# songrise/HyperNeRF-torch

Hardware: NVIDIA B200
Metric: train rays/s (fwd+bwd, 64+64 samples/ray, HyperNeRF warp+bendy-sheet) (higher is better)
Workload: dtype bf16

## Files before the change

hypernerf_torch_b200/csrc/hn_mlp.cu:

```cuda
#include <math.h>
#include <algorithm>
#include <string.h>
#include <type_traits>
#include <unordered_map>
#include "hn_api_internal.h"
#include "hn_mlp_program.h"
#include "hn_ptx.cuh"

#ifdef HN_MLP_FWD_VARIANT
namespace hn_fv { using namespace hn; }
#define hn hn_fv
#define hn_mlp_fwd hn_mlp_fwd_fv
#define hn_mlp_fwd_trunk hn_mlp_fwd_trunk_fv
#define HN_FV_HIDDEN __attribute__((visibility("hidden")))
#else
#define HN_FV_HIDDEN
#endif

namespace hn {

#ifndef HN_TRAP_IDS
#define HN_TRAP_IDS 1
#endif
#if HN_TRAP_IDS
// ... 806 lines not shown
          tc_fence_before();
          warp_arrive(my_ready);
        }
#if HN_ROLE_TIMING
        if (p.dbg && blockIdx.x == 0 && threadIdx.x == 0) {
          p.dbg[gridDim.x * 8 + li * 2] += t_drain - t_layer;
          p.dbg[gridDim.x * 8 + li * 2 + 1] += HN_T0() - t_drain;
        }
#endif
        (void)t_layer; (void)t_drain;
      }
    }
    if (p.dbg && threadIdx.x == 0) {
      const long long tt = HN_T0() - t_begin;
      p.dbg[blockIdx.x * 8 + 4] = t_acc; p.dbg[blockIdx.x * 8 + 5] = tt - t_acc - t_pro;
      p.dbg[blockIdx.x * 8 + 6] = t_pro; p.dbg[blockIdx.x * 8 + 7] = tt;
    }
    };
    if (kEpiSplit == 1 || share == 0) { setmaxnreg_inc<kRegsPrimary>(); epilogue(std::true_type{}); }
    else { setmaxnreg_dec<kRegsSecondary>(); epilogue(std::false_type{}); }
  }
  tc_fence_before();
  __syncthreads();
  if (warp == kIssuerWarp) tmem_dealloc(tmem_base, 256 * kSubTiles);
}

template <class C>
__device__ __forceinline__ void trunk_in_bwd(uint32_t tlane, const float* wp, float* gx) {
  if constexpr (C::KT <= 96) {
    float gf[C::KT];
#pragma unroll
    for (int c0 = 0; c0 < C::KT; c0 += 32) {
      uint32_t r[32];
      tmem_ld32(tlane + c0, r);
      tmem_ld_wait();
#pragma unroll
      for (int j = 0; j < 32; ++j) gf[c0 + j] = __uint_as_float(r[j]);
    }
    posenc_bwd<3, C::XF>(wp, gf, gx);
    if constexpr (C::H > 0) posenc_bwd<C::H, C::HF>(wp + 3, gf + C::PE_X, gx + 3);
  } else {
    static_assert(C::PE_X == 63, "the two-phase pull-back assumes the hyper block starts at column 63");
    float gh[C::PE_H + 8];
    {
      float ga[64];
#pragma unroll
      for (int c0 = 0; c0 < 64; c0 += 32) {
        uint32_t r[32];
        tmem_ld32(tlane + c0, r);
        tmem_ld_wait();
#pragma unroll
        for (int j = 0; j < 32; ++j) ga[c0 + j] = __uint_as_float(r[j]);
      }
      posenc_bwd<3, C::XF>(wp, ga, gx);
      gh[0] = ga[63];
    }
#pragma unroll
    for (int c0 = 64; c0 < C::KT; c0 += 16) {
      uint32_t r[16];
      tmem_ld16(tlane + c0, r);
      tmem_ld_wait();
#pragma unroll
      for (int j = 0; j < 16; ++j)
        if (c0 - 63 + j < C::PE_H) gh[c0 - 63 + j] = __uint_as_float(r[j]);
    }
    posenc_bwd<C::H, C::HF>(wp + 3, gh, gx + 3);
  }
}

template <class C>
__global__ void __launch_bounds__(kMlpThreads, 1) mlp_dgrad_kernel(const __grid_constant__ BwdParams p) {
  extern __shared__ __align__(1024) uint8_t smem[];
  using SM = SmemBwd<C>;
  using Ring = RingStateT<SM::STAGES>;
  constexpr bool PP = true;
  uint8_t* act = smem + SM::ACT;
  uint8_t* inb = smem + SM::INB;
  uint8_t* ring = smem + SM::RING;
  uint64_t* full = reinterpret_cast<uint64_t*>(smem + SM::BARS);
  uint64_t* empty = full + SM::STAGES;
  uint64_t* acc_full = empty + SM::STAGES;
  uint64_t* act_ready = acc_full + 2;
  uint32_t* tmem_ptr = reinterpret_cast<uint32_t*>(smem + SM::TMEMP);
  const int warp = threadIdx.x >> 5, lane = threadIdx.x & 31;

  if (threadIdx.x == 0) {
    for (int i = 0; i < SM::STAGES; ++i) { mbar_init(&full[i], 1); mbar_init(&empty[i], 1); }
    for (int i = 0; i < 2; ++i) { mbar_init(&acc_full[i], 1); mbar_init(&act_ready[i], 4 * Sched<PP>::SUBS * kEpiSplit); }
    fence_barrier_init();
  }
  if (warp == kIssuerWarp) { tmem_alloc(tmem_ptr, 256 * kSubTiles); tmem_relinquish(); }
  tc_fence_before();
  __syncthreads();
  tc_fence_after();
  const uint32_t tmem_base = *tmem_ptr;
  const Program& prog = p.prog;

  if (warp >= kEpiWarps) {
    setmaxnreg_dec<kRegsFeeder>();
    if (warp == kProducerWarp && lane == 0) {
      Ring rs;
      long long tw = 0;
      for (int tile = blockIdx.x; tile < p.n_tiles; tile += gridDim.x) produce_tile<PP>(prog, p.weights, ring, full, empty, rs, tw);
      if (p.dbg) p.dbg[blockIdx.x * 8 + 0] = tw;
    } else if (warp == kIssuerWarp) {
      Ring rs;
      uint32_t ph_ready = 0;
      long long t_ready = 0, t_full = 0;
      const long long t_begin = HN_T0();
      const uint32_t act_s = smem_u32(act), inb_s = smem_u32(inb), ring_s = smem_u32(ring);
      for (int tile = blockIdx.x; tile < p.n_tiles; tile += gridDim.x) {
        for (int li = 0; li < prog.nlayers; ++li) {
          for (int chain = 0; chain < Sched<PP>::CHAINS; ++chain) {
            long long t0 = HN_T0();
            mbar_wait(&act_ready[chain], ph_ready);
            t_ready += HN_T0() - t0;
            tc_fence_after();
            issue_layer<PP>(prog, prog.layers[li], chain * Sched<PP>::SUBS, act_s, inb_s, SM::ACT_BYTES, SM::INB_BYTES, ring_s, tmem_base,
                        full, empty, rs, t_full);
            if (elect_one_sync()) umma_commit(&acc_full[chain]);
            __syncwarp();
          }
          ph_ready ^= 1;
        }
      }
      if (p.dbg && lane == 0) {
        p.dbg[blockIdx.x * 8 + 1] = t_ready; p.dbg[blockIdx.x * 8 + 2] = t_full; p.dbg[blockIdx.x * 8 + 3] = HN_T0() - t_begin;
      }
    }
  } else {
    const int sub = warp / (4 * kEpiSplit);
    const int share = (warp >> 2) % kEpiSplit;
    const int quarter = warp & 3;
    auto epilogue = [&](auto primary_tag) {
    constexpr bool PRIMARY = decltype(primary_tag)::value;
    const int row = quarter * 32 + lane;
    const uint32_t tlane = tmem_base + ((uint32_t)(quarter * 32) << 16) + sub * 256;
    uint8_t* act_row = act + sub * SM::ACT_BYTES + row * 16;
    uint8_t* inb_row = inb + sub * SM::INB_BYTES + row * 16;
    const int chain = PP ? sub : 0;
    uint64_t* my_acc = &acc_full[chain];
    uint64_t* my_ready = &act_ready[chain];
    uint32_t ph_acc = 0;
    long long t_acc = 0, t_pro = 0;
    const long long t_begin = HN_T0();
    for (int tile = blockIdx.x; tile < p.n_tiles; tile += gridDim.x) {
      const long long t_tile = HN_T0();
      const int64_t g = (int64_t)tile * kCtaRows + sub * kTileRows + row;
      const bool valid = g < p.n;
      const int64_t gc = valid ? g : p.n - 1;
      const int64_t ray = gc / p.S;
      const int64_t gq = p.pos != nullptr ? ray * p.S_full + __ldg(p.pos + gc) : gc;
      const size_t half = (size_t)tile * (2 * kSubTiles) + sub * 2 + (row >> 6);
      const uint32_t* gate_row = p.gates + half * (size_t)p.g_total * kHalfRows + (row & 63);
      uint4* save_row = reinterpret_cast<uint4*>(p.dsaved + half * (size_t)p.d_total * kHalfChunkBytes) + (row & 63);

      if constexpr (PRIMARY) {
        float f[16];
#pragma unroll
        for (int i = 0; i < 16; ++i) f[i] = 0.f;
        if (valid) {
#pragma unroll
          for (int i = 0; i < 3; ++i) {
            float y = __ldg(p.rgb + gq * 3 + i);
            f[i] = __ldg(p.g_rgb + gq * 3 + i) * y * (1.f - y);
          }
        }
        store_features<16>(f, act_row, save_row, p.d_rgbhead);
        if constexpr (C::STATIC) {
#pragma unroll
          for (int i = 0; i < 16; ++i) f[i] = 0.f;
          if (valid && __ldg(p.sigma + gq) > 0.f) f[0] = __ldg(p.g_sigma + gq);
          store_features<16>(f, inb_row, save_row, p.d_sigma);
        }
      }
      fence_proxy_async_smem();
      tc_fence_before();
      warp_arrive(my_ready);
      t_pro += HN_T0() - t_tile;

      float gx_skip[C::STATIC ? 1 : C::NWARPED] = {};
      for (int li = 0; li < prog.nlayers; ++li) {
        const Layer& L = prog.layers[li];
        if (L.epi == BE_MASK) {
          if (L.n_out == kTrunkW) bwd_masked_share<kTrunkW>(share, tlane, gate_row, L.gate_word, act_row, save_row, L.save_chunk, my_acc, ph_acc, t_acc);
          else if (L.n_out == kWsW) bwd_masked_share<kWsW>(share, tlane, gate_row, L.gate_word, act_row, save_row, L.save_chunk, my_acc, ph_acc, t_acc);
          else bwd_masked_share<kRgbW>(share, tlane, gate_row, L.gate_word, act_row, save_row, L.save_chunk, my_acc, ph_acc, t_acc);
          fence_proxy_async_smem();
          if (li + 1 < prog.nlayers) { tc_fence_before(); warp_arrive(my_ready); }
          continue;
        }
        if (!C::STATIC && L.epi == BE_RGB1) {
          bwd_masked_share<kRgbW>(share, tlane, gate_row, L.gate_word, act_row, save_row, L.save_chunk, my_acc, ph_acc, t_acc);
          if constexpr (PRIMARY) {
          float f[16];
#pragma unroll
          for (int i = 0; i < 16; ++i) f[i] = 0.f;
          if (valid) f[0] = __ldg(p.g_sigma + gq) * (-expm1f(-__ldg(p.sigma + gq)));
          store_features<16>(f, act_row + (kRgbW / 8) * kChunkBytes, save_row, L.save_chunk + kRgbW / 8);
          }
          fence_proxy_async_smem(); tc_fence_before(); warp_arrive(my_ready);
          continue;
        }
        { long long t0 = HN_T0(); mbar_wait(my_acc, ph_acc); ph_acc ^= 1; t_acc += HN_T0() - t0; }
        tc_fence_after();
        if (L.epi == BE_LINEAR || L.epi == BE_LINCOND) {
          if (L.n_out == kTrunkW) bwd_linear_share<kTrunkW>(share, tlane, act_row, save_row, L.save_chunk);
          else bwd_linear_share<kRgbW>(share, tlane, act_row, save_row, L.save_chunk);
          if constexpr (PRIMARY && !C::STATIC) {
            if (L.epi == BE_LINCOND) {
              uint32_t r[16];
              tmem_ld16(tlane + kRgbW, r);
              tmem_ld_wait();
              float v[C::G];
#pragma unroll
              for (int i = 0; i < C::G; ++i) v[i] = __uint_as_float(r[i]);
              const int64_t id = __ldg(p.ids + ray);
              HN_CHECK_ID(id, p.n_embed);
              glo_grad_add<C::G>(v, valid, id, p.glo_grad, lane);
            }
          }
        } else if constexpr (PRIMARY && !C::STATIC) {
        if (L.epi == BE_SKIPSTORE || L.epi == BE_TRUNKIN) {
          float wp[C::NWARPED], gx[C::NWARPED];
          const int64_t gw = p.g_warped_out != nullptr ? gc : gq;
#pragma unroll
          for (int i = 0; i < C::NWARPED; ++i) wp[i] = __ldg(p.warped + gw * C::NWARPED + i);
          trunk_in_bwd<C>(tlane, wp, gx);
          if (L.epi == BE_SKIPSTORE) {
#pragma unroll
            for (int i = 0; i < C::NWARPED; ++i) gx_skip[i] = gx[i];
          } else if (p.g_warped_out != nullptr) {
            if (valid) {
#pragma unroll
              for (int i = 0; i < C::NWARPED; ++i) {
                float v = gx[i] + gx_skip[i];
                if (p.g_warped != nullptr) v += __ldg(p.g_warped + gq * C::NWARPED + i);
                p.g_warped_out[g * C::NWARPED + i] = v;
              }
            }
          } else if constexpr (!C::NOWARP) {
          float f[16];
#pragma unroll
          for (int i = 0; i < 16; ++i) f[i] = 0.f;
          if (valid) {
#pragma unroll
            for (int i = 0; i < C::NWARPED; ++i) {
              f[i] = gx[i] + gx_skip[i];
              if (p.g_warped != nullptr) f[i] += __ldg(p.g_warped + gq * C::NWARPED + i);
            }
          }
          if constexpr (C::H == C::G) {
            if (p.mflags & MF_AXIS) {
              const int64_t id = __ldg(p.ids + ray);
              glo_grad_add<C::G>(f + 3, valid, id, p.glo_grad, lane);
#pragma unroll
              for (int i = 0; i < C::G; ++i) f[3 + i] = 0.f;
            }
          }
          if constexpr (C::SE3) {
            float x[3], wv[6], gy[3];
#pragma unroll
            for (int i = 0; i < 3; ++i) { x[i] = __ldg(p.points + gq * 3 + i); gy[i] = f[i]; }
#pragma unroll
            for (int i = 0; i < 6; ++i) wv[i] = __ldg(p.aux + gc * 6 + i);
            se3_apply_bwd(x, wv, wv + 3, gy, f, f + 3);
          }
          store_features<16>(f, act_row, save_row, L.save_chunk);
          }
        } else if constexpr (!C::NOWARP) {
          uint32_t r[16];
          tmem_ld16(tlane + kWsW, r);
          tmem_ld_wait();
          float v[C::G];
#pragma unroll
          for (int i = 0; i < C::G; ++i) v[i] = __uint_as_float(r[i]);
          const int64_t id = __ldg(p.ids + ray);
          HN_CHECK_ID(id, p.n_embed);
          glo_grad_add<C::G>(v, valid, id, p.glo_grad, lane);
        }
        }
        if (li + 1 < prog.nlayers) {
          fence_proxy_async_smem();
          tc_fence_before();
          warp_arrive(my_ready);
        }
      }
    }
    if (p.dbg && threadIdx.x == 0) {
      const long long tt = HN_T0() - t_begin;
      p.dbg[blockIdx.x * 8 + 4] = t_acc; p.dbg[blockIdx.x * 8 + 5] = tt - t_acc - t_pro;
      p.dbg[blockIdx.x * 8 + 6] = t_pro; p.dbg[blockIdx.x * 8 + 7] = tt;
    }
    };
    if (kEpiSplit == 1 || share == 0) { setmaxnreg_inc<kRegsPrimary>(); epilogue(std::true_type{}); }
    else { setmaxnreg_dec<kRegsSecondary>(); epilogue(std::false_type{}); }
  }
  tc_fence_before();
  __syncthreads();
  if (warp == kIssuerWarp) tmem_dealloc(tmem_base, 256 * kSubTiles);
}

#ifndef HN_MLP_FWD_VARIANT
constexpr int kWgStages = 3;
constexpr int kWgStageA = 256 * kHalfChunkBytes / 8;
constexpr int kWgStageBytes = 2 * kWgStageA;
struct WgSmem {
  static constexpr int STAGES = 0;
  static constexpr int BARS = kWgStages * kWgStageBytes;
  static constexpr int TMEMP = BARS + (2 * kWgStages + 2) * 8;
  static constexpr int TOTAL = TMEMP + 16;
};
static int wgrad_groups(int njobs) { return njobs >= 24 ? 8 : 4; }
static void assign_wgrad_groups(WgradTable& t, int groups, int grid, int16_t* group_start) {
  int order[kMaxJobs];
  int64_t load[16] = {};
  auto cost = [&](int i) { return (int)t.jobs[i].dy_nchunks + t.jobs[i].x0_nchunks + t.jobs[i].x1_nchunks; };
  for (int i = 0; i < t.njobs; ++i) order[i] = i;
  std::stable_sort(order, order + t.njobs, [&](int a, int b) { return cost(a) > cost(b); });
  for (int k = 0; k < t.njobs; ++k) {
    int best = 0;
    for (int g = 1; g < groups; ++g) if (load[g] < load[best]) best = g;
    t.jobs[order[k]].group = (uint8_t)best;
    load[best] += cost(order[k]);
  }
  int ctas[16];
  for (int g = 0; g < groups; ++g) ctas[g] = 1;
  for (int c = groups; c < grid; ++c) {
    int best = 0;
    for (int g = 1; g < groups; ++g)
      if (load[g] * ctas[best] > load[best] * ctas[g]) best = g;
    ++ctas[best];
  }
  group_start[0] = 0;
  for (int g = 0; g < groups; ++g) group_start[g + 1] = (int16_t)(group_start[g] + ctas[g]);
}

__device__ __forceinline__ float pe_window(float alpha, uint8_t win_c, int e) {
  const int C = win_c & ~kWinIdentity;
  if (win_c & kWinIdentity) {
    if (e < C) return 1.f;
    e -= C;
  }
  const float x = fminf(fmaxf(alpha - (float)(e / (2 * C)), 0.f), 1.f);
  return 0.5f * (1.f - cospif(x));
}

struct WgradParams {
  WgradTable tab;
  const uint8_t* saved; const uint8_t* dsaved;
  const float* pe_alpha;
  float* flat_grad;
  int64_t n_half;
  int x_total, d_total;
  int groups;
  int16_t group_start[17];
};

template <bool WIN>
__global__ void __launch_bounds__(192, 1) mlp_wgrad_kernel(const __grid_constant__ WgradParams p) {
  extern __shared__ __align__(1024) uint8_t smem[];
  uint64_t* full = reinterpret_cast<uint64_t*>(smem + WgSmem::BARS);
  uint64_t* empty = full + kWgStages;
  uint64_t* acc_full = empty + kWgStages;
  uint64_t* acc_empty = acc_full + 1;
  uint32_t* tmem_ptr = reinterpret_cast<uint32_t*>(smem + WgSmem::TMEMP);
  const int warp = threadIdx.x >> 5, lane = threadIdx.x & 31;
  if (threadIdx.x == 0) {
    for (int i = 0; i < kWgStages; ++i) { mbar_init(&full[i], 1); mbar_init(&empty[i], 1 + 4); }
    mbar_init(acc_full, 1);
    mbar_init(acc_empty, 128);
    fence_barrier_init();
  }
  if (warp == 1) { tmem_alloc(tmem_ptr, 512); tmem_relinquish(); }
  tc_fence_before();
  __syncthreads();
  tc_fence_after();
  const uint32_t tmem_base = *tmem_ptr;

  int my_group = 0;
  while (my_group + 1 < p.groups && (int)blockIdx.x >= p.group_start[my_group + 1]) ++my_group;
  const int ctas_in_group = p.group_start[my_group + 1] - p.group_start[my_group];
  const int64_t per = (p.n_half + ctas_in_group - 1) / ctas_in_group;
  const int64_t h0 = (int64_t)((int)blockIdx.x - p.group_start[my_group]) * per;
  const int64_t h1 = min(h0 + per, p.n_half);
  const int njobs = p.tab.njobs;

  if (warp == 0) {
    if (lane == 0 && h0 < h1) {
      int slot = 0; uint32_t phase = 0;
      for (int ji = 0; ji < njobs; ++ji) {
        const WgradJob& J = p.tab.jobs[ji];
        if (J.group != my_group) continue;
        const uint32_t a_bytes = J.dy_nchunks * kHalfChunkBytes;
        const uint32_t b0_bytes = J.x0_nchunks * kHalfChunkBytes, b1_bytes = J.x1_nchunks * kHalfChunkBytes;
        for (int64_t h = h0; h < h1; ++h) {
          uint8_t* st = smem + slot * kWgStageBytes;
          mbar_wait(&empty[slot], phase ^ 1);
          mbar_arrive_expect_tx(&full[slot], a_bytes + b0_bytes + b1_bytes);
          bulk_g2s(st, p.dsaved + ((size_t)h * p.d_total + J.dy_chunk) * kHalfChunkBytes, a_bytes, &full[slot]);
          bulk_g2s(st + kWgStageA, p.saved + ((size_t)h * p.x_total + J.x0_chunk) * kHalfChunkBytes, b0_bytes, &full[slot]);
          if (b1_bytes)
            bulk_g2s(st + kWgStageA + b0_bytes, p.saved + ((size_t)h * p.x_total + J.x1_chunk) * kHalfChunkBytes, b1_bytes,
                       &full[slot]);
          if (++slot == kWgStages) { slot = 0; phase ^= 1; }
        }
      }
    }
  } else if (warp == 1) {
    if (h0 < h1) {
      int slot = 0; uint32_t phase = 0, ph_empty = 0;
      constexpr uint32_t kHi = (1u << 14) | (kHalfChunkBytes >> 4);
      const uint32_t st0 = smem_u32(smem);
      bool first = true;
      for (int ji = 0; ji < njobs; ++ji) {
        const WgradJob& J = p.tab.jobs[ji];
        if (J.group != my_group) continue;
        const uint32_t ncols = (J.x0_nchunks + J.x1_nchunks) * 8;
        const uint32_t idesc = make_idesc_bf16(128, ncols, 1, 1);
        const bool two = J.mblocks == 2;
        const uint32_t d1 = tmem_base + ncols;
        if (!first) { mbar_wait(acc_empty, ph_empty); ph_empty ^= 1; tc_fence_after(); }
        first = false;
        for (int64_t h = h0; h < h1; ++h) {
          mbar_wait(&full[slot], phase);
          tc_fence_after();
          if (elect_one_sync()) {
            const uint32_t a_lo = ((st0 + slot * kWgStageBytes) >> 4) | ((128u >> 4) << 16);
            const uint32_t b_lo = a_lo + (kWgStageA >> 4);
            uint32_t acc = h > h0;
#pragma unroll
            for (int ks = 0; ks < kHalfRows / 16; ++ks) {
              const uint64_t bd = ((uint64_t)kHi << 32) | (b_lo + ks * 16);
              umma_bf16(tmem_base, ((uint64_t)kHi << 32) | (a_lo + ks * 16), bd, idesc, acc);
              if (two) umma_bf16(d1, ((uint64_t)kHi << 32) | (a_lo + ks * 16 + ((16 * kHalfChunkBytes) >> 4)), bd, idesc, acc);
              acc = 1;
            }
            umma_commit(&empty[slot]);
          }
          __syncwarp();
          if (++slot == kWgStages) { slot = 0; phase ^= 1; }
        }
        if (elect_one_sync()) umma_commit(acc_full);
        __syncwarp();
      }
    }
  } else if (h0 < h1) {
    const int quarter = warp & 3;
    const int wr = warp - 2;
    const uint32_t tlane = tmem_base + ((uint32_t)(quarter * 32) << 16);
    int slot = 0; uint32_t phase = 0, ph_acc = 0;
    for (int ji = 0; ji < njobs; ++ji) {
      const WgradJob& J = p.tab.jobs[ji];
      if (J.group != my_group) continue;
      const int ncols = (J.x0_nchunks + J.x1_nchunks) * 8;
      const int cpw = (J.dy_nchunks + 3) / 4;
      const int c_lo = min(wr * cpw, (int)J.dy_nchunks), c_hi = min(c_lo + cpw, (int)J.dy_nchunks);
      float bs[8][8];
#pragma unroll
      for (int a = 0; a < 8; ++a)
#pragma unroll
        for (int b = 0; b < 8; ++b) bs[a][b] = 0.f;
      for (int64_t h = h0; h < h1; ++h) {
        mbar_wait(&full[slot], phase);
        if (J.nbias) {
          const uint8_t* st = smem + slot * kWgStageBytes;
#pragma unroll
          for (int a = 0; a < 8; ++a) {
            if (c_lo + a < c_hi) {
#pragma unroll
              for (int rr = 0; rr < kHalfRows; rr += 32) {
                uint4 v = *reinterpret_cast<const uint4*>(st + (c_lo + a) * kHalfChunkBytes + (rr + lane) * 16);
                bs[a][0] += bf16_lo(v.x); bs[a][1] += bf16_hi(v.x); bs[a][2] += bf16_lo(v.y); bs[a][3] += bf16_hi(v.y);
                bs[a][4] += bf16_lo(v.z); bs[a][5] += bf16_hi(v.z); bs[a][6] += bf16_lo(v.w); bs[a][7] += bf16_hi(v.w);
              }
            }
          }
        }
        __syncwarp();
        if (lane == 0) mbar_arrive(&empty[slot]);
        if (++slot == kWgStages) { slot = 0; phase ^= 1; }
      }
      if (J.nbias) {
#pragma unroll
        for (int a = 0; a < 8; ++a) {
          if (c_lo + a < c_hi) {
#pragma unroll
            for (int b = 0; b < 8; ++b) {
              float v = bs[a][b];
#pragma unroll
              for (int o = 16; o > 0; o >>= 1) v += __shfl_xor_sync(0xffffffffu, v, o);
              const int col = (c_lo + a) * 8 + b;
              if (lane == 0) {
                for (int s = 0; s < J.nbias; ++s) {
                  const BiasSeg& B = J.bias[s];
                  if (col >= B.col0 && col < B.col0 + B.ncols) atomicAdd(p.flat_grad + B.dst + (col - B.col0), v);
                }
              }
            }
          }
        }
      }
      mbar_wait(acc_full, ph_acc); ph_acc ^= 1;
      tc_fence_after();
      for (int mb = 0; mb < J.mblocks; ++mb) {
        const int drow = mb * 128 + quarter * 32 + lane;
        for (int c0 = 0; c0 < ncols; c0 += 16) {
          uint32_t r[16];
          tmem_ld16(tlane + mb * ncols + c0, r);
          tmem_ld_wait();
          for (int s = 0; s < J.nflush; ++s) {
            const FlushSeg& F = J.flush[s];
            if (drow >= F.row0 && drow < F.row0 + F.nrows) {
              float* dst = p.flat_grad + F.dst + (int64_t)(drow - F.row0) * F.ld + (c0 - (int)F.col0);
              const bool vec = (reinterpret_cast<uintptr_t>(dst) & 15) == 0;
              uint32_t v[16];
#pragma unroll
              for (int j = 0; j < 16; ++j) v[j] = r[j];
              if (WIN && F.win != kNoWin) {
                const float a = p.pe_alpha[F.win - 1];
#pragma unroll
                for (int j = 0; j < 16; ++j)
                  v[j] = __float_as_uint(__uint_as_float(r[j]) * pe_window(a, F.win_c, (int)F.win_e0 + c0 + j - (int)F.col0));
              }
#pragma unroll
              for (int j = 0; j < 16; j += 4) {
                const int col = c0 + j;
                if (vec && col >= F.col0 && col + 4 <= F.col0 + F.ncols) {
                  red_add_v4(dst + j, v[j], v[j + 1], v[j + 2], v[j + 3]);
                } else {
#pragma unroll
                  for (int jj = j; jj < j + 4; ++jj)
                    if (c0 + jj >= F.col0 && c0 + jj < F.col0 + F.ncols) atomicAdd(dst + jj, __uint_as_float(v[jj]));
                }
              }
            }
          }
        }
      }
      tc_fence_before();
      mbar_arrive(acc_empty);
    }
  }
  tc_fence_before();
  __syncthreads();
  if (warp == 1) tmem_dealloc(tmem_base, 512);
}

struct PackParams {
  PackTable tab;
  const float* flat;
  const float* pe_alpha;
  uint8_t* blob;
  int64_t bias_off, glo_off;
  int64_t glo_src;
  int glo_floats;
};

__global__ void pack_kernel(const __grid_constant__ PackParams p) {
  const int oi = blockIdx.y;
  if (oi < p.tab.nops) {
    const PackOp& op = p.tab.ops[oi];
    const int npk = op.n * (op.k / 8);
    for (int i = blockIdx.x * blockDim.x + threadIdx.x; i < npk; i += gridDim.x * blockDim.x) {
      const int chunk = i / op.n, n = i % op.n;
      float v[8];
#pragma unroll
      for (int j = 0; j < 8; ++j) v[j] = 0.f;
      for (int b = op.blk0; b < op.blk0 + op.nblk; ++b) {
        const PackBlock& B = p.tab.blocks[b];
        if (n < B.n0 || n >= B.n0 + B.nn) continue;
        const float a = p.pe_alpha != nullptr && B.win != kNoWin ? __ldg(p.pe_alpha + B.win - 1) : 0.f;
        const bool win = p.pe_alpha != nullptr && B.win != kNoWin;
#pragma unroll
        for (int j = 0; j < 8; ++j) {
          int k = chunk * 8 + j;
          if (k >= B.k0 && k < B.k0 + B.kk) {
            if (B.sk == kBiasPairStride) {
              const float bv = __ldg(p.flat + B.src + (int64_t)(n - B.n0) * B.sn);
              const float hi = __uint_as_float(pack_bf16(bv, 0.f) << 16);
              v[j] = k == B.k0 ? hi : bv - hi;
            } else {
              v[j] = __ldg(p.flat + B.src + (int64_t)(n - B.n0) * B.sn + (int64_t)(k - B.k0) * B.sk);
              if (win) v[j] *= pe_window(a, B.win_c, (int)B.win_e0 + (B.sk == 1 ? k - B.k0 : n - B.n0));
            }
          }
        }
      }
      uint4 o;
      o.x = pack_bf16(v[0], v[1]); o.y = pack_bf16(v[2], v[3]); o.z = pack_bf16(v[4], v[5]); o.w = pack_bf16(v[6], v[7]);
      reinterpret_cast<uint4*>(p.blob + (size_t)op.w_off16 * 16)[i] = o;
    }
  } else {
    float* bias = reinterpret_cast<float*>(p.blob + p.bias_off);
    for (int i = blockIdx.x * blockDim.x + threadIdx.x; i < p.tab.bias_floats; i += gridDim.x * blockDim.x) {
      float v = 0.f;
      for (int b = 0; b < p.tab.nbias; ++b) {
        const BiasBlock& B = p.tab.bias[b];
        if (i >= B.dst && i < B.dst + B.cnt) v = __ldg(p.flat + B.src + (i - B.dst));
      }
      bias[i] = v;
    }
    float* glo = reinterpret_cast<float*>(p.blob + p.glo_off);
    for (int i = blockIdx.x * blockDim.x + threadIdx.x; i < p.glo_floats; i += gridDim.x * blockDim.x)
      glo[i] = __ldg(p.flat + p.glo_src + i);
  }
}

#endif

static unsigned long long* g_dbg = nullptr;
static int64_t tiles_of(int64_t n) { return (n + kCtaRows - 1) / kCtaRows; }

template <class K, class P>
static cudaError_t launch_mlp(K kernel, int grid, int smem, cudaStream_t stream, const P& params) {
  kernel<<<grid, kMlpThreads, smem, stream>>>(params);
  return cudaGetLastError();
}

template <class K>
static int set_smem(K kernel, int bytes, const char* what) {
  static thread_local std::unordered_map<const void*, int> done;
  int dev = 0;
  if (cudaError_t e = cudaGetDevice(&dev)) return set_cuda_error(e, what);
  auto it = done.find((const void*)kernel);
  if (it != done.end() && it->second == dev) return 0;
  cudaError_t e = cudaFuncSetAttribute(kernel, cudaFuncAttributeMaxDynamicSharedMemorySize, bytes);
  if (e == cudaSuccess) done[(const void*)kernel] = dev;
  return set_cuda_error(e, what);
}

struct PlanCache {
  bool have_plan = false, have_tables = false, windowed = false;
  hn_model_desc desc;
  int level = -1;
  int64_t offs[HN_NUM_PARAM_TENSORS];
  ModelPlan plan;
};
static ModelPlan& cached_plan(const hn_model_desc& d, int level = -1, const int64_t* offsets = nullptr,
                              bool windowed = false) {
  static thread_local PlanCache c;
  if (!c.have_plan || memcmp(&c.desc, &d, sizeof(d)) != 0) {
    build_plan(d, &c.plan);
    c.desc = d; c.have_plan = true; c.have_tables = false;
  }
  if (offsets != nullptr) {
    const size_t nb = sizeof(int64_t) * c.plan.info.n_params;
    if (!c.have_tables || c.level != level || c.windowed != windowed || memcmp(c.offs, offsets, nb) != 0) {
      build_tables(d, level, offsets, windowed, &c.plan);
      memcpy(c.offs, offsets, nb);
      c.level = level; c.windowed = windowed; c.have_tables = true;
    }
  }
  return c.plan;
}

}

using namespace hn;

#ifndef HN_MLP_FWD_VARIANT
extern "C" int hn_query(const hn_model_desc* desc, int64_t n_samples, hn_sizes* out) {
  if (!desc || !out) return set_error(-2, "hn_query: null pointer");
  if (int rc = validate_desc(*desc)) return rc;
  if (n_samples < 0) return set_error(-1, "hn_query: negative n_samples");
  const ModelPlan& plan = cached_plan(*desc);
  memset(out, 0, sizeof(*out));
  const int64_t halves = 2 * kSubTiles * tiles_of(n_samples);
  out->packed_bytes = plan.layout.total;
  out->saved_bytes = halves * plan.info.x_total * kHalfChunkBytes + halves * plan.info.g_total * kHalfRows * 4;
  out->workspace_bytes = halves * plan.info.d_total * kHalfChunkBytes;
  const Dims& m = plan.dims;
  auto lin = [](int64_t out_f, int64_t in_f) { return out_f * in_f + out_f; };
  if (is_static(*desc)) {
    out->flat_param_floats = lin(kTrunkW, m.pe_x) + 6 * lin(kTrunkW, kTrunkW) + lin(kTrunkW, kTrunkW + m.pe_x) + lin(1, kTrunkW) +
                             lin(kTrunkW, kTrunkW) + lin(kRgbW, kTrunkW + m.pe_v) + lin(3, kRgbW);
    return 0;
  }
  int64_t cnt = plan.info.glo_floats;
  if (m.se3) {
    cnt += lin(kSe3W, m.in_w) + 4 * lin(kSe3W, kSe3W) + lin(kSe3W, kSe3W + m.in_w) + lin(kSe3W, kSe3W) +
           2 * (lin(kSe3W, kSe3W) + lin(3, kSe3W));
  } else if (!m.nowarp) {
    if (!m.axis) cnt += lin(kSheetW, m.in_s) + 4 * lin(kSheetW, kSheetW) + lin(kSheetW, kSheetW + m.in_s) + lin(m.H, kSheetW);
    cnt += lin(kWarpW, m.in_w) + 4 * lin(kWarpW, kWarpW) + lin(kWarpW, kWarpW + m.in_w) + lin(3, kWarpW);
  }
  int64_t lvl = lin(kTrunkW, m.in_t) + 7 * lin(kTrunkW, kTrunkW) + lin(kTrunkW, kTrunkW + m.in_t) + lin(kRgbW, kTrunkW) +
                lin(kRgbW, kRgbW + m.pe_v + (m.cond_r ? m.G : 0)) + 3 * lin(kRgbW, kRgbW) + lin(3, kRgbW) +
                lin(1, kRgbW + (m.cond_a ? m.G : 0));
  out->flat_param_floats = cnt + 2 * lvl;
  return 0;
}

static int pack_impl(const hn_model_desc* desc, const float* flat_params, const int64_t* param_offsets, int level,
                     void* packed, const float* pe_alpha, void* stream) {
  if (!desc || !flat_params || !param_offsets || !packed) return set_error(-2, "hn_pack_weights: null pointer");
  if (level < 0 || level > 1) return set_error(-1, "hn_pack_weights: level must be 0 or 1");
  if (int rc = validate_desc(*desc)) return rc;
  const ModelPlan& plan = cached_plan(*desc, level, param_offsets, pe_alpha != nullptr);
  PackParams pp;
  pp.tab = plan.pack;
  pp.flat = flat_params;
  pp.pe_alpha = pe_alpha;
  pp.blob = (uint8_t*)packed;
  pp.bias_off = plan.layout.bias_off;
  pp.glo_off = plan.layout.glo_off;
  pp.glo_src = plan.info.glo_param >= 0 ? param_offsets[plan.info.glo_param] : 0;
  if (plan.info.glo_param >= 0 && pp.glo_src < 0) return set_error(-2, "hn_pack_weights: the GLO table of this configuration has no offset");
  pp.glo_floats = plan.info.glo_floats;
  dim3 grid(16, plan.pack.nops + 1);
  pack_kernel<<<grid, 256, 0, (cudaStream_t)stream>>>(pp);
  return set_cuda_error(cudaGetLastError(), "hn_pack_weights");
}

extern "C" int hn_pack_weights(const hn_model_desc* desc, const float* flat_params, const int64_t* param_offsets, int level,
                               void* packed, void* stream) {
  return pack_impl(desc, flat_params, param_offsets, level, packed, nullptr, stream);
}

extern "C" int hn_pack_weights_windowed(const hn_model_desc* desc, const float* flat_params, const int64_t* param_offsets,
                                        int level, void* packed, const float* pe_alpha, void* stream) {
  if (!pe_alpha) return set_error(-2, "hn_pack_weights_windowed: null pe_alpha");
  if (desc && is_static(*desc)) return set_error(-13, "hn_pack_weights_windowed: the static NeRF has no encoding window");
  return pack_impl(desc, flat_params, param_offsets, level, packed, pe_alpha, stream);
}

#endif

static int model_flags(const hn_model_desc& d) {
  int f = 0;
  if (d.flags & HN_FLAG_SLICE_AXIS) f |= MF_AXIS;
  if (d.flags & (HN_FLAG_ALPHA_COND | HN_FLAG_RGB_COND)) f |= MF_COND;
  return f;
}
static int shape_of(const hn_model_desc& d) {
  if (is_static(d)) return 0;
  if (d.flags & HN_FLAG_WARP_SE3) return 5;
  if (!has_warp(d)) return 4;
  return d.hyper_dim == 2 ? 1 : d.hyper_dim == 4 ? 2 : 3;
}
#define HN_DISPATCH_SHAPE(shape, MACRO) \
  switch (shape) {                      \
    case 0: MACRO(CfgStatic); break;    \
    case 1: MACRO(Cfg1); break;         \
    case 2: MACRO(CfgH4); break;        \
    case 3: MACRO(CfgH8); break;        \
    case 5: MACRO(CfgSE3); break;       \
    default: MACRO(CfgT); break;        \
  }

template <class C, bool STASH>
static int launch_fwd(const FwdParams& fp, int grid, void* stream) {
  if (int rc = set_smem(mlp_fwd_kernel<C, STASH>, Smem<C>::TOTAL, "hn_mlp_fwd: smem attr")) return rc;
  return set_cuda_error(launch_mlp(mlp_fwd_kernel<C, STASH>, grid, Smem<C>::TOTAL, (cudaStream_t)stream, fp), "hn_mlp_fwd");
}

static int mlp_fwd_impl(const hn_model_desc* desc, const void* packed, const float* points, const float* warped_in,
                        const float* viewdirs, const int64_t* ids, const float* noise, float noise_std, int64_t B, int S,
                        const int32_t* pos, int S_full, float* sigma, float* rgb, float* warped, void* saved, float* aux,
                        void* stream) {
  if (!desc || !packed || (!points && !warped_in) || !viewdirs || !sigma || !rgb) return set_error(-2, "hn_mlp_fwd: null pointer");
  if (B < 0 || S <= 0) return set_error(-1, "hn_mlp_fwd: bad B/S");
  if (pos != nullptr && S_full < S) return set_error(-1, "hn_mlp_fwd: scattered rows need S_full >= S");
  if (int rc = validate_desc(*desc)) return rc;
  const bool stat = is_static(*desc);
  const int mflags = stat ? 0 : model_flags(*desc);
  if (!stat && !has_warp(*desc) && !warped_in) { warped_in = points; warped = nullptr; }
  const bool trunk = warped_in != nullptr;
  if (!stat && (desc->flags & HN_FLAG_WARP_SE3) && !trunk && saved != nullptr && !aux)
    return set_error(-2, "hn_mlp_fwd: the SE3 warp needs the aux buffer when the stash is written");
  if (trunk && stat) return set_error(-13, "hn_mlp_fwd_trunk: the static model has no warp / sheet stage to skip");
  if (!stat && !ids && (!trunk || (mflags & MF_COND))) return set_error(-2, "hn_mlp_fwd: null ids");
  if (B == 0) return 0;
  const ModelPlan& plan = cached_plan(*desc);
  FwdParams fp;
  const bool train = saved != nullptr;
  fp.prog = trunk ? (train ? plan.fwd_trunk_train : plan.fwd_trunk) : (train ? plan.fwd_train : plan.fwd);
  fp.warped_in = warped_in;
  fp.weights = (const uint8_t*)packed + plan.layout.fwd_off;
  fp.bias = (const float*)((const uint8_t*)packed + plan.layout.bias_off);
  fp.glo = (const float*)((const uint8_t*)packed + plan.layout.glo_off);
  fp.points = points; fp.viewdirs = viewdirs; fp.ids = ids; fp.noise = noise; fp.noise_std = noise_std;
  fp.n = B * S; fp.S = S; fp.n_embed = desc->num_embeddings;
  fp.view_freqs = desc->view_freqs; fp.mflags = mflags;
// ... 210 lines not shown
```

Before: 674,500.

## Use variable-size slot ring for weight-gradient TMA pipeline

Replaces the fixed 3-stage double-size buffers in the weight-gradient kernel with a 7-slot ring of half-size slots. A stage takes one slot when dy and x chunks fit together, otherwise two consecutive slots, tracked with per-slot phase bits. The aim is to keep more loads in flight for small jobs within the same shared memory, which deepens the producer/MMA pipeline. It adds per-slot phase bookkeeping and extra barrier waits and arrivals for two-slot stages, and is correct only if every warp role computes the same slot sequence.

```diff
diff --git a/hypernerf_torch_b200/csrc/hn_mlp.cu b/hypernerf_torch_b200/csrc/hn_mlp.cu
--- a/hypernerf_torch_b200/csrc/hn_mlp.cu
+++ b/hypernerf_torch_b200/csrc/hn_mlp.cu
@@ -1132,15 +1132,22 @@
 }
 
 #ifndef HN_MLP_FWD_VARIANT
-constexpr int kWgStages = 3;
-constexpr int kWgStageA = 256 * kHalfChunkBytes / 8;
-constexpr int kWgStageBytes = 2 * kWgStageA;
+constexpr int kWgSlots = 7;
+constexpr int kWgSlotBytes = 256 * kHalfChunkBytes / 8;
 struct WgSmem {
-  static constexpr int STAGES = 0;
-  static constexpr int BARS = kWgStages * kWgStageBytes;
-  static constexpr int TMEMP = BARS + (2 * kWgStages + 2) * 8;
+  static constexpr int BARS = kWgSlots * kWgSlotBytes;
+  static constexpr int TMEMP = BARS + (2 * kWgSlots + 2) * 8;
   static constexpr int TOTAL = TMEMP + 16;
 };
+static_assert(WgSmem::TOTAL <= 227 * 1024, "weight-gradient ring exceeds the shared memory of a block");
+struct WgStage {
+  int s, xs, n;
+  uint32_t xoff;
+};
+__device__ __forceinline__ WgStage wg_stage(int s, uint32_t a_bytes, uint32_t b_bytes) {
+  if (a_bytes + b_bytes <= (uint32_t)kWgSlotBytes) return {s, s, 1, a_bytes};
+  return {s, s + 1 == kWgSlots ? 0 : s + 1, 2, 0u};
+}
 static int wgrad_groups(int njobs) { return njobs >= 24 ? 8 : 4; }
 static void assign_wgrad_groups(WgradTable& t, int groups, int grid, int16_t* group_start) {
   int order[kMaxJobs];
@@ -1191,13 +1198,13 @@
 __global__ void __launch_bounds__(192, 1) mlp_wgrad_kernel(const __grid_constant__ WgradParams p) {
   extern __shared__ __align__(1024) uint8_t smem[];
   uint64_t* full = reinterpret_cast<uint64_t*>(smem + WgSmem::BARS);
-  uint64_t* empty = full + kWgStages;
-  uint64_t* acc_full = empty + kWgStages;
+  uint64_t* empty = full + kWgSlots;
+  uint64_t* acc_full = empty + kWgSlots;
   uint64_t* acc_empty = acc_full + 1;
   uint32_t* tmem_ptr = reinterpret_cast<uint32_t*>(smem + WgSmem::TMEMP);
   const int warp = threadIdx.x >> 5, lane = threadIdx.x & 31;
   if (threadIdx.x == 0) {
-    for (int i = 0; i < kWgStages; ++i) { mbar_init(&full[i], 1); mbar_init(&empty[i], 1 + 4); }
+    for (int i = 0; i < kWgSlots; ++i) { mbar_init(&full[i], 1); mbar_init(&empty[i], 1 + 4); }
     mbar_init(acc_full, 1);
     mbar_init(acc_empty, 128);
     fence_barrier_init();
@@ -1218,28 +1225,31 @@
 
   if (warp == 0) {
     if (lane == 0 && h0 < h1) {
-      int slot = 0; uint32_t phase = 0;
+      int s = 0; uint32_t ebits = 0;
       for (int ji = 0; ji < njobs; ++ji) {
         const WgradJob& J = p.tab.jobs[ji];
         if (J.group != my_group) continue;
         const uint32_t a_bytes = J.dy_nchunks * kHalfChunkBytes;
         const uint32_t b0_bytes = J.x0_nchunks * kHalfChunkBytes, b1_bytes = J.x1_nchunks * kHalfChunkBytes;
         for (int64_t h = h0; h < h1; ++h) {
-          uint8_t* st = smem + slot * kWgStageBytes;
-          mbar_wait(&empty[slot], phase ^ 1);
-          mbar_arrive_expect_tx(&full[slot], a_bytes + b0_bytes + b1_bytes);
-          bulk_g2s(st, p.dsaved + ((size_t)h * p.d_total + J.dy_chunk) * kHalfChunkBytes, a_bytes, &full[slot]);
-          bulk_g2s(st + kWgStageA, p.saved + ((size_t)h * p.x_total + J.x0_chunk) * kHalfChunkBytes, b0_bytes, &full[slot]);
+          const WgStage S = wg_stage(s, a_bytes, b0_bytes + b1_bytes);
+          mbar_wait(&empty[S.s], ((ebits >> S.s) & 1) ^ 1);
+          ebits ^= 1u << S.s;
+          if (S.n == 2) { mbar_wait(&empty[S.xs], ((ebits >> S.xs) & 1) ^ 1); ebits ^= 1u << S.xs; }
+          mbar_arrive_expect_tx(&full[S.s], a_bytes + b0_bytes + b1_bytes);
+          bulk_g2s(smem + S.s * kWgSlotBytes, p.dsaved + ((size_t)h * p.d_total + J.dy_chunk) * kHalfChunkBytes, a_bytes,
+                   &full[S.s]);
+          uint8_t* xb = smem + S.xs * kWgSlotBytes + S.xoff;
+          bulk_g2s(xb, p.saved + ((size_t)h * p.x_total + J.x0_chunk) * kHalfChunkBytes, b0_bytes, &full[S.s]);
           if (b1_bytes)
-            bulk_g2s(st + kWgStageA + b0_bytes, p.saved + ((size_t)h * p.x_total + J.x1_chunk) * kHalfChunkBytes, b1_bytes,
-                       &full[slot]);
-          if (++slot == kWgStages) { slot = 0; phase ^= 1; }
+            bulk_g2s(xb + b0_bytes, p.saved + ((size_t)h * p.x_total + J.x1_chunk) * kHalfChunkBytes, b1_bytes, &full[S.s]);
+          s = S.xs + 1 == kWgSlots ? 0 : S.xs + 1;
         }
       }
     }
   } else if (warp == 1) {
     if (h0 < h1) {
-      int slot = 0; uint32_t phase = 0, ph_empty = 0;
+      int s = 0; uint32_t fbits = 0, ph_empty = 0;
       constexpr uint32_t kHi = (1u << 14) | (kHalfChunkBytes >> 4);
       const uint32_t st0 = smem_u32(smem);
       bool first = true;
@@ -1250,14 +1260,17 @@
         const uint32_t idesc = make_idesc_bf16(128, ncols, 1, 1);
         const bool two = J.mblocks == 2;
         const uint32_t d1 = tmem_base + ncols;
+        const uint32_t a_bytes = J.dy_nchunks * kHalfChunkBytes, b_bytes = (J.x0_nchunks + J.x1_nchunks) * kHalfChunkBytes;
         if (!first) { mbar_wait(acc_empty, ph_empty); ph_empty ^= 1; tc_fence_after(); }
         first = false;
         for (int64_t h = h0; h < h1; ++h) {
-          mbar_wait(&full[slot], phase);
+          const WgStage S = wg_stage(s, a_bytes, b_bytes);
+          mbar_wait(&full[S.s], (fbits >> S.s) & 1);
+          fbits ^= 1u << S.s;
           tc_fence_after();
           if (elect_one_sync()) {
-            const uint32_t a_lo = ((st0 + slot * kWgStageBytes) >> 4) | ((128u >> 4) << 16);
-            const uint32_t b_lo = a_lo + (kWgStageA >> 4);
+            const uint32_t a_lo = ((st0 + S.s * kWgSlotBytes) >> 4) | ((128u >> 4) << 16);
+            const uint32_t b_lo = ((st0 + S.xs * kWgSlotBytes + S.xoff) >> 4) | ((128u >> 4) << 16);
             uint32_t acc = h > h0;
 #pragma unroll
             for (int ks = 0; ks < kHalfRows / 16; ++ks) {
@@ -1266,10 +1279,11 @@
               if (two) umma_bf16(d1, ((uint64_t)kHi << 32) | (a_lo + ks * 16 + ((16 * kHalfChunkBytes) >> 4)), bd, idesc, acc);
               acc = 1;
             }
-            umma_commit(&empty[slot]);
+            umma_commit(&empty[S.s]);
+            if (S.n == 2) umma_commit(&empty[S.xs]);
           }
           __syncwarp();
-          if (++slot == kWgStages) { slot = 0; phase ^= 1; }
+          s = S.xs + 1 == kWgSlots ? 0 : S.xs + 1;
         }
         if (elect_one_sync()) umma_commit(acc_full);
         __syncwarp();
@@ -1279,11 +1293,12 @@
     const int quarter = warp & 3;
     const int wr = warp - 2;
     const uint32_t tlane = tmem_base + ((uint32_t)(quarter * 32) << 16);
-    int slot = 0; uint32_t phase = 0, ph_acc = 0;
+    int s = 0; uint32_t fbits = 0, ph_acc = 0;
     for (int ji = 0; ji < njobs; ++ji) {
       const WgradJob& J = p.tab.jobs[ji];
       if (J.group != my_group) continue;
       const int ncols = (J.x0_nchunks + J.x1_nchunks) * 8;
+      const uint32_t a_bytes = J.dy_nchunks * kHalfChunkBytes, b_bytes = (J.x0_nchunks + J.x1_nchunks) * kHalfChunkBytes;
       const int cpw = (J.dy_nchunks + 3) / 4;
       const int c_lo = min(wr * cpw, (int)J.dy_nchunks), c_hi = min(c_lo + cpw, (int)J.dy_nchunks);
       float bs[8][8];
@@ -1292,9 +1307,11 @@
 #pragma unroll
         for (int b = 0; b < 8; ++b) bs[a][b] = 0.f;
       for (int64_t h = h0; h < h1; ++h) {
-        mbar_wait(&full[slot], phase);
+        const WgStage S = wg_stage(s, a_bytes, b_bytes);
+        mbar_wait(&full[S.s], (fbits >> S.s) & 1);
+        fbits ^= 1u << S.s;
         if (J.nbias) {
-          const uint8_t* st = smem + slot * kWgStageBytes;
+          const uint8_t* st = smem + S.s * kWgSlotBytes;
 #pragma unroll
           for (int a = 0; a < 8; ++a) {
             if (c_lo + a < c_hi) {
@@ -1308,8 +1325,11 @@
           }
         }
         __syncwarp();
-        if (lane == 0) mbar_arrive(&empty[slot]);
-        if (++slot == kWgStages) { slot = 0; phase ^= 1; }
+        if (lane == 0) {
+          mbar_arrive(&empty[S.s]);
+          if (S.n == 2) mbar_arrive(&empty[S.xs]);
+        }
+        s = S.xs + 1 == kWgSlots ? 0 : S.xs + 1;
       }
       if (J.nbias) {
 #pragma unroll
```

Result: no change. 671,600 (median of 6 runs) (-0.4%).
